# LuckyLYM/Zebra

Hardware: AMD Instinct MI355X
Metric: temporal edges/sec embedded (k=20, 2-layer) (higher is better)
Workload: dtype f64+f32

## Files before the change

zebra_amd/csrc/aggregate.hip:

```cpp
#include "common.hpp"
#include "embed_out_body.hpp"
#include "fc1_tile.hpp"

using namespace zt;
using namespace zt::dense;

namespace {

constexpr int MAX_MT = 5;
constexpr int MAX_MT_BIG = 16;
constexpr int MAX_MT_BIG_WIDE = 8;

#ifdef ZT_AGG_STAMP
__device__ unsigned long long g_agg[8];
#define AGG_STAMP(i) do { if (threadIdx.x == 0) { const long long t__ = clock64(); atomicAdd(&g_agg[i], (unsigned long long)(t__ - t_prev__)); t_prev__ = t__; } } while (0)
#else
#define AGG_STAMP(i) do { } while (0)
#endif

template <bool TAB, int MMT = MAX_MT, int NW = NTW>
__global__ __launch_bounds__(AGG_THREADS) void k_fc1_agg(FcAggArgs a, int rq, int mt_count, int lda)
{
    extern __shared__ __attribute__((aligned(16))) char smem[];
    const float *__restrict__ memory = a.memory, *__restrict__ efeat = a.efeat, *__restrict__ overlay = a.overlay;
// ... 154 lines not shown
#pragma unroll
    for (int b = 0; b < NB; ++b)
#pragma unroll
        for (int j = 0; j < 3; ++j)
            bre[b][j] = j < nrem ? bp[(size_t)b * 64 * K1p - 4 * g4 + 16 * nchunk + 4 * j + g4] : 0.f;
    const float *ap = A + (size_t)r16 * lda + 4 * g4;
    for (int kc = 0; kc < nchunk; ++kc) {
        if (kc + 1 < nchunk) {
#pragma unroll
            for (int b = 0; b < NB; ++b) bnext[b] = *reinterpret_cast<const f32x4 *>(bp + (size_t)b * 64 * K1p + 16 * (kc + 1));
        }
        f32x4 av[5];
#pragma unroll
        for (int a = 0; a < 5; ++a) av[a] = *reinterpret_cast<const f32x4 *>(ap + (size_t)a * 16 * lda + 16 * kc);
#pragma unroll
        for (int j = 0; j < 4; ++j)
#pragma unroll
            for (int a = 0; a < 5; ++a)
#pragma unroll
                for (int b = 0; b < NB; ++b)
                    acc[a][b] = __builtin_amdgcn_mfma_f32_16x16x4f32(av[a][j], bcur[b][j], acc[a][b], 0, 0, 0);
#pragma unroll
        for (int b = 0; b < NB; ++b) bcur[b] = bnext[b];
    }
    const float *ar = A + (size_t)r16 * lda + 16 * nchunk + g4;
#pragma unroll
    for (int j = 0; j < 3; ++j) {
        if (j >= nrem) break;
        float av[5];
#pragma unroll
        for (int a = 0; a < 5; ++a) av[a] = ar[(size_t)a * 16 * lda + 4 * j];
#pragma unroll
        for (int a = 0; a < 5; ++a)
#pragma unroll
            for (int b = 0; b < NB; ++b)
                acc[a][b] = __builtin_amdgcn_mfma_f32_16x16x4f32(av[a], bre[b][j], acc[a][b], 0, 0, 0);
    }
}

template <int KK>
__global__ __launch_bounds__(AGG_THREADS, 4) void k_fc1_agg_d100(
    const float *__restrict__ P, const float *__restrict__ efeat, const float *__restrict__ time_w, long long num_nodes,
    long long num_edges, int F, long long N, int lda, const int *__restrict__ nbr, const int *__restrict__ eix,
    const float *__restrict__ dt, const float *__restrict__ w, const float *__restrict__ W1p, int K1p,
    const float *__restrict__ b1, float *__restrict__ H, float *__restrict__ S, int *status)
{
    constexpr int D = 100, T = 100, DP = 112, ROWS = 80, RQ = ROWS / KK, LDH = DP + 1;
    static_assert(ROWS % KK == 0, "a tile holds whole query rows");
    extern __shared__ __attribute__((aligned(16))) char smem[];
    float *A = reinterpret_cast<float *>(smem);
    float *wn = A + (size_t)ROWS * lda;
    float *wnn = wn + ROWS;
    int *g_nb = reinterpret_cast<int *>(wnn + ROWS);
    int *g_ei = g_nb + ROWS;
    float *g_dt = reinterpret_cast<float *>(g_ei + ROWS);
    const int tid = threadIdx.x, lane = tid & 63, wave = tid >> 6;
    const int r16 = lane & 15, g4 = lane >> 4;
    const int m = blockIdx.y;
    const long long q0 = (long long)blockIdx.x * RQ;
    const int nq = (int)((N - q0) < RQ ? (N - q0) : RQ);
    const int rows = nq * KK;
    const size_t mb = ((size_t)m * N + q0) * KK;
#ifdef ZT_AGG_STAMP
    long long t_prev__ = clock64();
#endif

    float ef1 = 0.f;
    if (tid < ROWS) {
        int nb = 0, ei = 0;
        float d = 0.f, wv = 0.f;
        if (tid < rows) {
            nb = nbr[mb + tid]; ei = eix[mb + tid]; d = dt[mb + tid]; wv = w[mb + tid];
            if (nb < 0 || nb >= num_nodes || ei < 0 || ei >= num_edges) {
                atomicExch(status, ZT_ERR_RANGE);
                nb = 0; ei = 0;
            }
            if (F == 1) ef1 = efeat[ei];
        }
        g_nb[tid] = nb; g_ei[tid] = ei; g_dt[tid] = d; wn[tid] = wv;
    }
    const int cc = tid & 127;
    const float wc = cc < T ? time_w[cc] : 0.f;
    const int col0 = wave * 16 + r16;
    const float bias0 = col0 < D ? b1[col0] : 0.f, bias1 = (wave < 3 && col0 + 64 < D) ? b1[col0 + 64] : 0.f;
    __syncthreads();
    AGG_STAMP(0);

    f32x4 acc[5][2];
#pragma unroll
    for (int a = 0; a < 5; ++a) {
        const int nb4[4] = {g_nb[a * 16 + g4 * 4 + 0], g_nb[a * 16 + g4 * 4 + 1], g_nb[a * 16 + g4 * 4 + 2], g_nb[a * 16 + g4 * 4 + 3]};
#pragma unroll
        for (int j = 0; j < 4; ++j) {
            const float *pr = P + (size_t)nb4[j] * DP + col0;
            acc[a][0][j] = pr[0];
            acc[a][1][j] = pr[wave < 3 ? 64 : 0];
        }
    }
    if (tid < ROWS) {
        const int q = tid / KK;
        float my_sum = 0.f;
#pragma unroll
        for (int j = 0; j < KK; ++j) my_sum += wn[q * KK + j];
        wnn[tid] = (my_sum == 0.f) ? 0.f : wn[tid] / my_sum;
        if (tid < rows && tid - q * KK == 0) S[(size_t)m * N + q0 + q] = (my_sum == 0.f) ? 0.f : 1.f;
    }
    AGG_STAMP(1);
    if (F == 1) {
        if (tid < ROWS) A[(size_t)tid * lda] = ef1;
    } else if (F > 0) {
        constexpr int GU = 8;
        const bool vecF = (F & 3) == 0 && ((size_t)efeat & 15) == 0;
        if (vecF) {
            const int F4 = F >> 2;
            const unsigned mF4 = fastdiv_magic((unsigned)F4);
            for (int f0 = tid; f0 < ROWS * F4; f0 += AGG_THREADS * GU) {
                f32x4 v[GU];
#pragma unroll
                for (int u = 0; u < GU; ++u) {
                    const int f = f0 + u * AGG_THREADS;
                    const int g = fastdiv(f, mF4), c = f - g * F4;
                    v[u] = (f < ROWS * F4 && g < rows) ? *reinterpret_cast<const f32x4 *>(efeat + (size_t)g_ei[g] * F + 4 * c)
                                                      : f32x4{0.f, 0.f, 0.f, 0.f};
                }
#pragma unroll
                for (int u = 0; u < GU; ++u) {
                    const int f = f0 + u * AGG_THREADS;
                    const int g = fastdiv(f, mF4), c = f - g * F4;
                    if (f < ROWS * F4) *reinterpret_cast<f32x4 *>(A + (size_t)g * lda + 4 * c) = v[u];
                }
            }
        } else {
            const unsigned mF = fastdiv_magic((unsigned)F);
            for (int f0 = tid; f0 < ROWS * F; f0 += AGG_THREADS * GU) {
                float v[GU];
#pragma unroll
                for (int u = 0; u < GU; ++u) {
                    const int f = f0 + u * AGG_THREADS;
                    const int g = fastdiv(f, mF), c = f - g * F;
                    v[u] = (f < ROWS * F && g < rows) ? efeat[(size_t)g_ei[g] * F + c] : 0.f;
                }
#pragma unroll
                for (int u = 0; u < GU; ++u) {
                    const int f = f0 + u * AGG_THREADS;
                    const int g = fastdiv(f, mF), c = f - g * F;
                    if (f < ROWS * F) A[(size_t)g * lda + c] = v[u];
                }
            }
        }
    }
    {
        const int g0 = (tid >> 7) * 40;
        const bool is_cos = cc < T;
        if (is_cos || F + cc < K1p) {
            float *dst = A + (size_t)g0 * lda + F + cc;
            float xmax = 0.f;
#pragma unroll 2
            for (int i = 0; i < 40; i += 4) {
                const f32x4 d4 = *reinterpret_cast<const f32x4 *>(g_dt + g0 + i);
#pragma unroll
                for (int u = 0; u < 4; ++u) {
                    const float x = d4[u] * wc;
                    xmax = fmaxf(xmax, fabsf(x));
                    dst[(size_t)(i + u) * lda] = time_cosf_fast(x);
                }
            }
            if (!is_cos) {
                for (int i = 0; i < 40; ++i) dst[(size_t)i * lda] = 0.f;
            } else if (!(xmax < 4.0e6f)) {
                for (int i = 0; i < 40; ++i) dst[(size_t)i * lda] = time_cosf(g_dt[g0 + i] * wc);
            }
        }
    }
    AGG_STAMP(2);
    AGG_STAMP(3);
    __syncthreads();
    AGG_STAMP(4);

    {
        const float *bp = W1p + (size_t)col0 * K1p + 4 * g4;
        const int K4 = (F + T + 3) & ~3, nchunk = K4 >> 4, nrem = (K4 & 15) >> 2;
        if (wave < 3) d100_mfma<2>(A, lda, bp, K1p, nchunk, nrem, r16, g4, acc);
        else          d100_mfma<1>(A, lda, bp, K1p, nchunk, nrem, r16, g4, acc);
    }
    AGG_STAMP(5);
    __syncthreads();

    float *Hs = A;
    {
        float *hp = Hs + (size_t)(g4 * 4) * LDH + col0;
#pragma unroll
        for (int a = 0; a < 5; ++a) {
            const f32x4 w4 = *reinterpret_cast<const f32x4 *>(wnn + a * 16 + g4 * 4);
#pragma unroll
            for (int j = 0; j < 4; ++j) {
                float v = acc[a][0][j] + bias0;
                v = v > 0.f ? v : 0.f;
                hp[(size_t)(a * 16 + j) * LDH] = v * w4[j];
            }
        }
        if (wave < 3) {
#pragma unroll
            for (int a = 0; a < 5; ++a) {
                const f32x4 w4 = *reinterpret_cast<const f32x4 *>(wnn + a * 16 + g4 * 4);
#pragma unroll
                for (int j = 0; j < 4; ++j) {
                    float v1 = acc[a][1][j] + bias1;
                    v1 = v1 > 0.f ? v1 : 0.f;
                    hp[(size_t)(a * 16 + j) * LDH + 64] = v1 * w4[j];
                }
            }
        }
    }
    __syncthreads();
    AGG_STAMP(6);
    if (cc < D) {
        for (int q = tid >> 7; q < nq; q += 2) {
            const float *hq = Hs + (size_t)(q * KK) * LDH + cc;
            float s = 0.f;
#pragma unroll
            for (int j = 0; j < KK; ++j) s += hq[(size_t)j * LDH];
            H[((size_t)m * N + q0 + q) * D + cc] = s;
        }
    }
    AGG_STAMP(7);
}

#ifdef ZT_DIAG
__device__ unsigned long long g_regclk[4 * 1024];
#endif
constexpr int REG_NS = 26;
constexpr int REG_NB = 7;
constexpr int REG_FRAG_GROUPS = (REG_NB * REG_NS + 3) / 4;

__global__ void k_pack_reg_frag(const float *__restrict__ W1t, int K2p, float *__restrict__ image)
{
    const int i = blockIdx.x * blockDim.x + threadIdx.x;
    if (i >= REG_FRAG_GROUPS * 64 * 4) return;
    const int e = i & 3, lane = (i >> 2) & 63, G = i >> 8;
    const int q = 4 * G + e, b = q / REG_NS, st = q % REG_NS;
    image[i] = q < REG_NB * REG_NS ? W1t[(16 * b + (lane & 15)) * K2p + 4 * st + (lane >> 4)] : 0.f;
}

template <int KK, int DBG = 0>
__global__ __launch_bounds__(AGG_THREADS, 1) void k_fc1_agg_reg(
    const float *__restrict__ P, const float *__restrict__ efeat, const float *__restrict__ time_w, long long num_nodes,
    long long num_edges, int F, long long N, int M, const int *__restrict__ nbr, const int *__restrict__ eix,
    const float *__restrict__ dt, const float *__restrict__ w, const float *__restrict__ Wfrag,
    const float *__restrict__ b1, float *__restrict__ H, float *__restrict__ S, int *status,
    const int *gate_word, int gate_target, int *gate_latch)
{
    constexpr int D = 100, T = 100, DP = 112, ROWS = 80, RQ = ROWS / KK;
    static_assert(KK % 4 == 0 && ROWS % KK == 0, "groups of 4 rows must not straddle query rows");
    __shared__ int s_nb[AGG_WAVES][ROWS];
    __shared__ __attribute__((aligned(16))) float s_dt[AGG_WAVES][ROWS];
    __shared__ __attribute__((aligned(16))) float s_w[AGG_WAVES][ROWS];
    __shared__ float s_sum[AGG_WAVES][4];
    __shared__ __attribute__((aligned(16))) float s_ef[AGG_WAVES][ROWS * 4];
    const int lane = threadIdx.x & 63, wave = threadIdx.x >> 6;
    const int r16 = lane & 15, g4 = lane >> 4;
    int *nb_s = s_nb[wave];
    float *dt_s = s_dt[wave], *w_s = s_w[wave], *sum_s = s_sum[wave], *ef_s = s_ef[wave];
#ifdef ZT_DIAG
    const unsigned long long wall_in = DBG ? __builtin_amdgcn_s_memrealtime() : 0ull;
#endif

    float Breg[REG_NB][REG_NS];
    {
        const f32x4 *Wf = reinterpret_cast<const f32x4 *>(Wfrag) + lane;
        static_assert(REG_FRAG_GROUPS % 2 == 0, "two batches");
        constexpr int HB = REG_FRAG_GROUPS / 2;
#pragma unroll
        for (int half = 0; half < 2; ++half) {
            f32x4 v[HB];
#pragma unroll
            for (int i = 0; i < HB; ++i) v[i] = Wf[(half * HB + i) * 64];
            __builtin_amdgcn_sched_barrier(0);
#pragma unroll
            for (int i = 0; i < HB; ++i)
#pragma unroll
                for (int e = 0; e < 4; ++e) {
                    const int q = 4 * (half * HB + i) + e;
                    if (q < REG_NB * REG_NS) asm volatile("v_accvgpr_write_b32 %0, %1" : "=a"(Breg[q / REG_NS][q % REG_NS]) : "v"(v[i][e]));
                }
            __builtin_amdgcn_sched_barrier(0);
        }
    }
    float freq[REG_NS];
#pragma unroll
    for (int st = 0; st < REG_NS; ++st) {
        const int kc = 4 * st + g4 - F;
        freq[st] = (kc >= 0 && kc < T) ? time_w[kc] : 0.f;
    }
    float bias[REG_NB];
#pragma unroll
    for (int b = 0; b < REG_NB; ++b) bias[b] = (16 * b + r16) < D ? b1[16 * b + r16] : 0.f;

#ifdef ZT_DIAG
    const unsigned long long clk0 = DBG ? __builtin_amdgcn_s_memtime() : 0ull, wall0 = DBG ? __builtin_amdgcn_s_memrealtime() : 0ull;
#endif
    const long long tpm = (N + RQ - 1) / RQ;
    const long long n_tiles = tpm * M;
    const long long stride = (long long)gridDim.x * AGG_WAVES;
    long long tile = (long long)blockIdx.x * AGG_WAVES + wave;

    int pf_nb[2] = {0, 0}, pf_ei[2] = {0, 0};
    float pf_dt[2] = {0.f, 0.f}, pf_w[2] = {0.f, 0.f};
    auto fetch = [&](long long t) {
        const long long m = t / tpm, q0 = (t - m * tpm) * RQ;
        const int rows = (int)((N - q0) < RQ ? (N - q0) : RQ) * KK;
        const size_t mb = ((size_t)m * N + q0) * KK;
#pragma unroll
        for (int h = 0; h < 2; ++h) {
            const int row = h * 64 + lane;
            const bool in = row < rows && (h == 0 || lane < ROWS - 64);
            pf_nb[h] = in ? nbr[mb + row] : 0;
            pf_ei[h] = in ? eix[mb + row] : 0;
            pf_dt[h] = in ? dt[mb + row] : 0.f;
            pf_w[h] = in ? w[mb + row] : 0.f;
        }
    };
    float pf_ef[2][4] = {{0.f, 0.f, 0.f, 0.f}, {0.f, 0.f, 0.f, 0.f}};
    auto fetch_ef = [&]() {
#pragma unroll
        for (int h = 0; h < 2; ++h) {
            const int ei = pf_ei[h];
            const bool ok = ei >= 0 && ei < num_edges && (h == 0 || lane < ROWS - 64);
#pragma unroll
            for (int c = 0; c < 4; ++c) pf_ef[h][c] = (ok && c < F) ? efeat[(size_t)ei * F + c] : 0.f;
        }
    };
    member_gate_enter(gate_word, gate_target, status, gate_latch);
    if (tile < n_tiles) { fetch(tile); fetch_ef(); }

#pragma nounroll
    for (; tile < n_tiles; tile += stride) {
        const long long m = tile / tpm, q0 = (tile - m * tpm) * RQ;
        const int nq = (int)((N - q0) < RQ ? (N - q0) : RQ);
#pragma unroll
        for (int h = 0; h < 2; ++h) {
            const int row = h * 64 + lane;
            if (h == 0 || lane < ROWS - 64) {
                int nb = pf_nb[h], ei = pf_ei[h];
                if (nb < 0 || nb >= num_nodes || ei < 0 || ei >= num_edges) { atomicExch(status, ZT_ERR_RANGE); nb = 0; ei = 0; }
                nb_s[row] = nb; dt_s[row] = pf_dt[h]; w_s[row] = pf_w[h];
                *reinterpret_cast<f32x4 *>(ef_s + 4 * row) = f32x4{pf_ef[h][0], pf_ef[h][1], pf_ef[h][2], pf_ef[h][3]};
            }
        }
        wave_sync();
        if (lane < RQ) {
            f32x4 wv[KK / 4];
#pragma unroll
            for (int j = 0; j < KK / 4; ++j) wv[j] = *reinterpret_cast<const f32x4 *>(w_s + lane * KK + 4 * j);
            float sm = 0.f;
#pragma unroll
            for (int j = 0; j < KK; ++j) sm += wv[j / 4][j % 4];
            sum_s[lane] = sm;
            if (lane < nq) S[(size_t)m * N + q0 + lane] = (sm == 0.f) ? 0.f : 1.f;
        }
        wave_sync();
#pragma unroll
        for (int h = 0; h < 2; ++h) {
            const int row = h * 64 + lane;
            if (h == 0 || lane < ROWS - 64) {
                const float qs = sum_s[row / KK];
                w_s[row] = (qs == 0.f) ? 0.f : pf_w[h] / qs;
            }
        }
        wave_sync();
        const bool has_next = tile + stride < n_tiles;
        if (has_next) fetch(tile + stride);

        float Hloc[RQ][REG_NB];
#pragma unroll
        for (int q = 0; q < RQ; ++q)
#pragma unroll
            for (int b = 0; b < REG_NB; ++b) Hloc[q][b] = 0.f;

        f32x4 acc[REG_NB];
        float accv[REG_NB][4], Pv[2][REG_NB][4], wn_cur[4], wn_prv[4];
        auto load_P = [&](int x) {
            const int4 nb4 = *reinterpret_cast<const int4 *>(nb_s + x * 16 + 4 * g4);
            const float *p0 = P + (size_t)nb4.x * DP + r16, *p1 = P + (size_t)nb4.y * DP + r16,
                        *p2 = P + (size_t)nb4.z * DP + r16, *p3 = P + (size_t)nb4.w * DP + r16;
#pragma unroll
            for (int b = 0; b < REG_NB; ++b) {
                Pv[x & 1][b][0] = p0[16 * b]; Pv[x & 1][b][1] = p1[16 * b]; Pv[x & 1][b][2] = p2[16 * b]; Pv[x & 1][b][3] = p3[16 * b];
            }
        };
        if (!(DBG & 4)) { load_P(0); load_P(1); }
#pragma unroll
        for (int a = 0; a <= 5; ++a) {
            float dta = 0.f, A_next[2] = {0.f, 0.f};
            if (a > 0) {
#pragma unroll
                for (int b = 0; b < REG_NB; ++b)
#pragma unroll
                    for (int j = 0; j < 4; ++j) accv[b][j] = acc[b][j];
#pragma unroll
                for (int j = 0; j < 4; ++j) wn_prv[j] = wn_cur[j];
            }
            if (a < 5) {
                dta = dt_s[a * 16 + r16];
                const float ef = ef_s[4 * (a * 16 + r16) + (g4 & 3)];
                const f32x4 w4 = *reinterpret_cast<const f32x4 *>(w_s + a * 16 + 4 * g4);
#pragma unroll
                for (int j = 0; j < 4; ++j) wn_cur[j] = w4[j];
#pragma unroll
                for (int b = 0; b < REG_NB; ++b) acc[b] = f32x4{bias[b], bias[b], bias[b], bias[b]};
                A_next[0] = (DBG & 1) ? dta * freq[0] : time_cosf_rev(dta * freq[0]);
                A_next[1] = (DBG & 1) ? dta * freq[1] : time_cosf_rev(dta * freq[1]);
                if (g4 < F) A_next[0] = ef;
                if (a == 2 && has_next) fetch_ef();
            }
            __builtin_amdgcn_sched_barrier(0);
            const int ap = a > 0 ? a - 1 : 0;
            const int q_lo = (16 * ap) / KK, q_hi = (16 * ap + 15) / KK;
#pragma unroll
            for (int st0 = 0; st0 < REG_NS; st0 += 2) {
                if (a == 5 && st0 >= REG_NB) break;
                const float A_cur[2] = {A_next[0], A_next[1]};
                if (a < 5) {
#pragma unroll
                    for (int u = 0; u < 2; ++u)
                        if (st0 + 2 + u < REG_NS)
                            A_next[u] = (DBG & 1) ? dta * freq[st0 + 2 + u] : time_cosf_rev(dta * freq[st0 + 2 + u]);
#pragma unroll
                    for (int u = 0; u < 2; ++u)
#pragma unroll
                        for (int b = 0; b < REG_NB; ++b)
                            acc[b] = __builtin_amdgcn_mfma_f32_16x16x4f32(A_cur[u], Breg[b][st0 + u], acc[b], 0, 0, 0);
                }
#pragma unroll
                for (int u = 0; u < 2; ++u) {
                    const int st = st0 + u;
                    if (!(a > 0 && st < REG_NB)) continue;
                    const int b = st;
                    float part = 0.f;
#pragma unroll
                    for (int j = 0; j < 4; ++j) {
                        float v = accv[b][j] + ((DBG & 2) ? 0.f : Pv[ap & 1][b][j]);
                        v = v > 0.f ? v : 0.f;
                        part += (DBG & 2) ? v : v * wn_prv[j];
                    }
                    if (DBG & 2) {
                        Hloc[q_lo][b] += part;
                    } else {
                        const int pi = __float_as_int(part);
                        const auto h = __builtin_amdgcn_permlane32_swap(pi, pi, false, false);
                        const auto lo = __builtin_amdgcn_permlane16_swap(h[0], h[0], false, false);
                        const auto hi = __builtin_amdgcn_permlane16_swap(h[1], h[1], false, false);
                        const float pg[4] = {__int_as_float(lo[0]), __int_as_float(lo[1]), __int_as_float(hi[0]), __int_as_float(hi[1])};
#pragma unroll
                        for (int g = 0; g < 4; ++g) {
                            const int q = (16 * ap + 4 * g) / KK;
                            if (q < RQ) Hloc[q][b] += pg[g];
                        }
                    }
                    asm volatile("" : "+v"(Hloc[q_lo][b]));
                    if (q_hi != q_lo && q_hi < RQ) asm volatile("" : "+v"(Hloc[q_hi][b]));
                }
                if (a >= 1 && a <= 3 && st0 == REG_NB + 1 && !(DBG & 4)) load_P(a + 1);
                __builtin_amdgcn_sched_barrier(0);
            }
        }
#pragma unroll
        for (int q = 0; q < RQ; ++q) {
            if (g4 == (q & 3) && q < nq) {
                float *hrow = H + ((size_t)m * N + q0 + q) * D;
#pragma unroll
                for (int b = 0; b < REG_NB; ++b)
                    if (16 * b + r16 < D) hrow[16 * b + r16] = Hloc[q][b];
            }
        }
        wave_sync();
    }
#ifdef ZT_DIAG
    if (DBG && lane == 0 && blockIdx.x * AGG_WAVES + wave < 1024) {
        unsigned long long *o = g_regclk + 4 * (blockIdx.x * AGG_WAVES + wave);
        o[0] = __builtin_amdgcn_s_memtime() - clk0; o[1] = wall0; o[2] = __builtin_amdgcn_s_memrealtime();
        o[3] = wall_in;
    }
#endif
}


constexpr int EO3_NT = 7, EO3_KC = 7, EO3_DP = 112, EO3_LDY = 116;
constexpr int EO3_FRAG = EO3_NT * EO3_KC * 256;

__device__ __forceinline__ void eo3_fill(float *Wl, const float *__restrict__ Wp, int tid)
{
    constexpr int PER = (EO3_NT * EO3_KC * 64 + 255) / 256;
    f32x4 v[PER];
#pragma unroll
    for (int q = 0; q < PER; ++q) {
        const int idx = tid + q * 256, frag = idx >> 6, ln = idx & 63;
        const int b = frag / EO3_KC, c = frag - b * EO3_KC;
        v[q] = idx < EO3_NT * EO3_KC * 64
                   ? *reinterpret_cast<const f32x4 *>(Wp + (size_t)(16 * b + (ln & 15)) * EO3_DP + 16 * c + 4 * (ln >> 4))
                   : f32x4{0.f, 0.f, 0.f, 0.f};
    }
#pragma unroll
    for (int q = 0; q < PER; ++q) {
        const int idx = tid + q * 256;
        if (idx < EO3_NT * EO3_KC * 64) reinterpret_cast<f32x4 *>(Wl)[idx] = v[q];
    }
}

template <int HG>
__global__ __launch_bounds__(AGG_THREADS, 1) void k_embed_out3(
    const float *__restrict__ memory, long long num_nodes, const int *__restrict__ nodes, long long N, int D, int M,
    const float *__restrict__ H, const float *__restrict__ S, const float *__restrict__ fc2_p,
    const float *__restrict__ fc2_b, const float *__restrict__ fc1s_p, const float *__restrict__ fc1s_b,
    const float *__restrict__ fc2s_p, const float *__restrict__ fc2s_b, float *__restrict__ out, int *status, int n_src)
{
    extern __shared__ __attribute__((aligned(16))) char smem[];
    float *W0 = reinterpret_cast<float *>(smem);
    const int tid = threadIdx.x, lane = tid & 63, wave = tid >> 6, r16 = lane & 15, g4 = lane >> 4;
    const int OW = D * (M + 1);
    const long long tiles = (N + 15) / 16;
    const f32x4 zero4 = {0.f, 0.f, 0.f, 0.f};
    bool cin[EO3_KC];
#pragma unroll
    for (int c = 0; c < EO3_KC; ++c) cin[c] = 16 * c + 4 * g4 < D;
    const f32x4 *Wf0 = reinterpret_cast<const f32x4 *>(W0) + lane;

    if ((int)blockIdx.x < n_src) {
        float *W1 = W0 + EO3_FRAG;
        float *Y = W1 + EO3_FRAG + wave * 16 * EO3_LDY;
        eo3_fill(W0, fc1s_p, tid);
        eo3_fill(W1, fc2s_p, tid);
        float b1v[EO3_NT], b2v[EO3_NT];
#pragma unroll
        for (int b = 0; b < EO3_NT; ++b) {
            b1v[b] = 16 * b + r16 < D ? fc1s_b[16 * b + r16] : 0.f;
            b2v[b] = 16 * b + r16 < D ? fc2s_b[16 * b + r16] : 0.f;
        }
        const f32x4 *Wf1 = reinterpret_cast<const f32x4 *>(W1) + lane;
        const long long stride = (long long)n_src * AGG_WAVES;
        long long t = (long long)blockIdx.x * AGG_WAVES + wave;
        auto node_of = [&](long long tt) -> int { return (tt < tiles && tt * 16 + r16 < N) ? nodes[tt * 16 + r16] : -1; };
        auto rows_of = [&](int nd, f32x4 (&a)[EO3_KC]) {
            const bool ok = nd >= 0 && nd < num_nodes;
#pragma unroll
            for (int c = 0; c < EO3_KC; ++c)
                a[c] = (ok && cin[c]) ? *reinterpret_cast<const f32x4 *>(memory + (size_t)nd * D + 16 * c + 4 * g4) : zero4;
        };
        int nd_cur = node_of(t), nd_nxt = node_of(t + stride);
        f32x4 a[EO3_KC], an[EO3_KC];
        if (t < tiles) rows_of(nd_cur, a);
        __syncthreads();
        for (; t < tiles; t += stride) {
            const long long r0 = t * 16;
            if (r0 + r16 < N && (nd_cur < 0 || nd_cur >= num_nodes)) atomicExch(status, ZT_ERR_RANGE);
            rows_of(nd_nxt, an);
            nd_cur = nd_nxt;
            nd_nxt = node_of(t + 2 * stride);
            f32x4 acc1[EO3_NT];
#pragma unroll
            for (int b = 0; b < EO3_NT; ++b) acc1[b] = zero4;
#pragma unroll
            for (int c = 0; c < EO3_KC; ++c) {
                f32x4 w[EO3_NT];
#pragma unroll
                for (int b = 0; b < EO3_NT; ++b) w[b] = Wf0[(b * EO3_KC + c) * 64];
#pragma unroll
                for (int j = 0; j < 4; ++j)
#pragma unroll
                    for (int b = 0; b < EO3_NT; ++b) acc1[b] = __builtin_amdgcn_mfma_f32_16x16x4f32(a[c][j], w[b][j], acc1[b], 0, 0, 0);
            }
#pragma unroll
            for (int b = 0; b < EO3_NT; ++b)
#pragma unroll
                for (int j = 0; j < 4; ++j) {
                    const float v = acc1[b][j] + b1v[b];
                    Y[(4 * g4 + j) * EO3_LDY + 16 * b + r16] = (16 * b + r16 < D && v > 0.f) ? v : 0.f;
                }
            wave_sync();
            f32x4 acc[EO3_NT];
#pragma unroll
            for (int b = 0; b < EO3_NT; ++b) acc[b] = zero4;
#pragma unroll
            for (int c = 0; c < EO3_KC; ++c) {
                const f32x4 y = *reinterpret_cast<const f32x4 *>(Y + r16 * EO3_LDY + 16 * c + 4 * g4);
                f32x4 w[EO3_NT];
#pragma unroll
                for (int b = 0; b < EO3_NT; ++b) w[b] = Wf1[(b * EO3_KC + c) * 64];
#pragma unroll
                for (int j = 0; j < 4; ++j)
#pragma unroll
                    for (int b = 0; b < EO3_NT; ++b) acc[b] = __builtin_amdgcn_mfma_f32_16x16x4f32(y[j], w[b][j], acc[b], 0, 0, 0);
            }
#pragma unroll
            for (int b = 0; b < EO3_NT; ++b) {
                const int col = 16 * b + r16;
                if (col < D) {
#pragma unroll
                    for (int j = 0; j < 4; ++j)
                        if (r0 + 4 * g4 + j < N) out[(size_t)(r0 + 4 * g4 + j) * OW + col] = acc[b][j] + b2v[b];
                }
            }
            wave_sync();
#pragma unroll
            for (int c = 0; c < EO3_KC; ++c) a[c] = an[c];
        }
        return;
    }
    eo3_fill(W0, fc2_p, tid);
    float b2v[EO3_NT];
#pragma unroll
    for (int b = 0; b < EO3_NT; ++b) b2v[b] = 16 * b + r16 < D ? fc2_b[16 * b + r16] : 0.f;
    const long long units = tiles * M;
    const long long stride = (long long)((int)gridDim.x - n_src) * AGG_WAVES;
    long long u = (long long)((int)blockIdx.x - n_src) * AGG_WAVES + wave;
    constexpr int GQ = HG == 1 ? 1 : 5;
    auto rows_of = [&](long long uu, int q0, f32x4 (&g)[GQ][EO3_KC]) {
        const long long m = uu / tiles, r = (uu - m * tiles) * 16 + r16;
        const bool rin = uu < units && r < N;
        const float *hp = H + (((size_t)m * N + (rin ? r : 0)) * HG + q0) * D + 4 * g4;
#pragma unroll
        for (int q = 0; q < GQ; ++q)
#pragma unroll
            for (int c = 0; c < EO3_KC; ++c) g[q][c] = (rin && cin[c]) ? *reinterpret_cast<const f32x4 *>(hp + (size_t)q * D + 16 * c) : zero4;
    };
    f32x4 gn[GQ][EO3_KC];
    if (HG == 1) rows_of(u, 0, gn);
    __syncthreads();
    for (; u < units; u += stride) {
        const long long m = u / tiles, r0 = (u - m * tiles) * 16;
        f32x4 a[EO3_KC];
        if (HG == 1) {
#pragma unroll
            for (int c = 0; c < EO3_KC; ++c) a[c] = gn[0][c];
        } else {
#pragma nounroll
            for (int q0 = 0; q0 < HG; q0 += GQ) {
                rows_of(u, q0, gn);
#pragma unroll
                for (int c = 0; c < EO3_KC; ++c) {
                    if (q0 == 0) a[c] = gn[0][c]; else a[c] += gn[0][c];
#pragma unroll
                    for (int q = 1; q < GQ; ++q) a[c] += gn[q][c];
                }
            }
        }
        float sv[4];
#pragma unroll
        for (int j = 0; j < 4; ++j) sv[j] = r0 + 4 * g4 + j < N ? S[(size_t)m * N + r0 + 4 * g4 + j] : 0.f;
        if (HG == 1) rows_of(u + stride, 0, gn);
        f32x4 acc[EO3_NT];
#pragma unroll
        for (int b = 0; b < EO3_NT; ++b) acc[b] = zero4;
#pragma unroll
        for (int c = 0; c < EO3_KC; ++c) {
            f32x4 w[EO3_NT];
#pragma unroll
            for (int b = 0; b < EO3_NT; ++b) w[b] = Wf0[(b * EO3_KC + c) * 64];
#pragma unroll
            for (int j = 0; j < 4; ++j)
#pragma unroll
                for (int b = 0; b < EO3_NT; ++b) acc[b] = __builtin_amdgcn_mfma_f32_16x16x4f32(a[c][j], w[b][j], acc[b], 0, 0, 0);
        }
#pragma unroll
        for (int b = 0; b < EO3_NT; ++b) {
            const int col = 16 * b + r16;
            if (col < D) {
#pragma unroll
                for (int j = 0; j < 4; ++j)
                    if (r0 + 4 * g4 + j < N) out[(size_t)(r0 + 4 * g4 + j) * OW + (size_t)D * (m + 1) + col] = acc[b][j] + b2v[b] * sv[j];
            }
        }
    }
}

template <int NW = NTW>
__global__ __launch_bounds__(AGG_THREADS) void k_project_rows(const float *__restrict__ memory, long long num_nodes,
                                                              int D, const float *__restrict__ Wm_p,
                                                              const int *__restrict__ rows, const int *__restrict__ count,
                                                              long long n_max, float *__restrict__ P)
{
    extern __shared__ __attribute__((aligned(16))) char smem[];
    const int Dp = (D + 15) / 16 * 16, ldx = Dp + 4, NT = Dp / 16;
    float *X = reinterpret_cast<float *>(smem);
    int *rid = reinterpret_cast<int *>(X + OUT_ROWS * ldx);
    const int tid = threadIdx.x, lane = tid & 63, wave = tid >> 6;
    const int r16 = lane & 15, g4 = lane >> 4;
    const long long r0 = (long long)blockIdx.x * OUT_ROWS;
    long long n = n_max;
    if (count != nullptr) { const long long c = *count; n = c < n ? c : n; }
    if (r0 >= n) return;
    if (tid < OUT_ROWS) {
        long long v = -1;
        if (r0 + tid < n) v = rows != nullptr ? (long long)rows[r0 + tid] : r0 + tid;
        rid[tid] = (v >= 0 && v < num_nodes) ? (int)v : -1;
    }
    __syncthreads();
    const unsigned mL = fastdiv_magic((unsigned)ldx);
    for (int f = tid; f < OUT_ROWS * ldx; f += AGG_THREADS) {
        const int g = fastdiv(f, mL), c = f - g * ldx;
        X[f] = (rid[g] >= 0 && c < D) ? memory[(size_t)rid[g] * D + c] : 0.f;
    }
    __syncthreads();
    f32x4 acc[OUT_MT][NW];
    small_gemm(X, ldx, Wm_p, Dp, NT, wave, lane, acc);
#pragma unroll
    for (int b = 0; b < NW; ++b) {
        const int col = (wave + b * AGG_WAVES) * 16 + r16;
        if (col >= Dp) continue;
#pragma unroll
        for (int a = 0; a < OUT_MT; ++a)
#pragma unroll
            for (int j = 0; j < 4; ++j) {
                const int g = a * 16 + g4 * 4 + j;
                if (rid[g] >= 0) P[(size_t)rid[g] * Dp + col] = acc[a][b][j];
            }
    }
}

struct EmbedPlan {
    int Dp, K1p, lda, mt, rq;
    size_t lds;
    int K2p, lda2, mt2, rq2;
    size_t lds2;
    size_t off_w1p, off_H, off_S, off_fc2t, off_fc1st, off_fc2st, off_w1t, off_wm, off_wl, off_wfrag, total;
    int hg;
};

bool tile_shape(int Kp, int Dp, int k, int T, int *lda_out, int *mt_out, int *rq_out, size_t *lds_out, int max_mt = MAX_MT)
{
    const int lda = Kp + 4;
    int mt = max_mt;
    while (mt > 1 && ((size_t)mt * 16 * lda * 4 + (size_t)mt * 16 * 16) > (size_t)AGG_LDS_BUDGET) --mt;
    int rq = (mt * 16) / k;
    if (rq < 1) {
        mt = (k + 15) / 16;
        rq = 1;
        if (mt > max_mt || ((size_t)mt * 16 * lda * 4 + (size_t)mt * 16 * 16) > (size_t)AGG_LDS_BUDGET) return false;
    }
    mt = (rq * k + 15) / 16;
    if ((size_t)mt * 16 * (Dp + 1) * 4 > (size_t)mt * 16 * lda * 4) return false;
    *lda_out = lda; *mt_out = mt; *rq_out = rq;
    *lds_out = (size_t)mt * 16 * lda * 4 + (size_t)mt * 16 * 16 + (size_t)T * 4;
    return true;
}

bool split_fits(int D, int F, int T, int k) { return k <= ZT_MAX_K_WIDE && fc1_agg_split_rows(D, F, T) > 0; }

bool make_plan(int64_t N, int D, int F, int T, int M, int k, EmbedPlan &p)
{
    if (!width_supported(D)) return false;
    const int K1 = D + F + T;
    p.Dp = round_up(D, 16);
    p.K1p = round_up(K1, 16);
    const bool big = k > MAX_MT * 16;
    const int max_mt = big ? (p.Dp > 16 * NTW * AGG_WAVES ? MAX_MT_BIG_WIDE : MAX_MT_BIG) : MAX_MT;
    const bool full_ok = tile_shape(p.K1p, p.Dp, k, T, &p.lda, &p.mt, &p.rq, &p.lds, max_mt);
    if (!full_ok) { p.mt = 0; p.rq = 1; p.lda = p.K1p + 4; p.lds = 0; }
    p.K2p = round_up(F + T, 16);
    p.mt2 = 0;
    if (!(full_ok || big) || !tile_shape(p.K2p, p.Dp, k, T, &p.lda2, &p.mt2, &p.rq2, &p.lds2, max_mt)) p.mt2 = 0;
    if (p.mt == 0 && p.mt2 == 0 && !split_fits(D, F, T, k)) return false;
    size_t o = 0;
    auto take = [&](size_t bytes) { size_t r = o; o += (bytes + 255) & ~(size_t)255; return r; };
    p.off_w1p = take((size_t)p.Dp * p.K1p * 4);
    p.off_fc2t = take((size_t)p.Dp * p.Dp * 4);
    p.off_fc1st = take((size_t)p.Dp * p.Dp * 4);
    p.off_fc2st = take((size_t)p.Dp * p.Dp * 4);
    p.off_w1t = take((size_t)p.Dp * p.K2p * 4);
    p.off_wm = take((size_t)p.Dp * p.Dp * 4);
    p.hg = fc1_agg_wide_supported(D, F, T, k) ? k / 4 : 1;
    p.off_wl = take(p.hg > 1 ? fc1_agg_wide_weight_bytes() : 0);
    p.off_wfrag = take((size_t)REG_FRAG_GROUPS * 64 * 4 * 4);
    p.off_H = take((size_t)M * N * D * 4 * p.hg);
    p.off_S = take((size_t)M * N * 4);
    p.total = o;
    return true;
}

// ... 399 lines not shown
```

Before: 14.07 million.

## Software-pipeline register aggregation kernel: stagger acc handoff, split P loads, drop divisions

Restructures the register-resident fc1 aggregation loop into a compile-time-unrolled per-subtile lambda. The next subtile's time encoding and row reads are computed during the current MFMA chain, accumulators are handed off piecewise, and neighbor P loads are spread across stages. Per-tile 64-bit divisions for m/q0 are replaced by incremental tile/row-base counters, and edge-feature loads become branchless, using unsigned range checks with clamped indices. The aim is to hide latency and cut scalar/ALU overhead, at the cost of more complex scheduling and possible register pressure.

```diff
diff --git a/zebra_amd/csrc/aggregate.hip b/zebra_amd/csrc/aggregate.hip
--- a/zebra_amd/csrc/aggregate.hip
+++ b/zebra_amd/csrc/aggregate.hip
@@ -480,14 +480,23 @@
     const long long tpm = (N + RQ - 1) / RQ;
     const long long n_tiles = tpm * M;
     const long long stride = (long long)gridDim.x * AGG_WAVES;
-    long long tile = (long long)blockIdx.x * AGG_WAVES + wave;
+    long long tile = (long long)blockIdx.x * AGG_WAVES + __builtin_amdgcn_readfirstlane(wave);
+    long long cur_t = tile, cur_rb = tile * RQ;
+    const long long rb_wrap = N - tpm * RQ;
+    if (tile < n_tiles)
+        while (cur_t >= tpm) { cur_t -= tpm; cur_rb += rb_wrap; }
+    long long nxt_t = cur_t, nxt_rb = cur_rb;
+    auto advance = [&](long long &t, long long &rb) {
+        t += stride; rb += stride * RQ;
+        while (t >= tpm) { t -= tpm; rb += rb_wrap; }
+    };
 
     int pf_nb[2] = {0, 0}, pf_ei[2] = {0, 0};
     float pf_dt[2] = {0.f, 0.f}, pf_w[2] = {0.f, 0.f};
-    auto fetch = [&](long long t) {
-        const long long m = t / tpm, q0 = (t - m * tpm) * RQ;
+    auto fetch = [&](long long t, long long rb) {
+        const long long q0 = t * RQ;
         const int rows = (int)((N - q0) < RQ ? (N - q0) : RQ) * KK;
-        const size_t mb = ((size_t)m * N + q0) * KK;
+        const size_t mb = (size_t)rb * KK;
 #pragma unroll
         for (int h = 0; h < 2; ++h) {
             const int row = h * 64 + lane;
@@ -499,30 +508,36 @@
         }
     };
     float pf_ef[2][4] = {{0.f, 0.f, 0.f, 0.f}, {0.f, 0.f, 0.f, 0.f}};
-    auto fetch_ef = [&]() {
-#pragma unroll
-        for (int h = 0; h < 2; ++h) {
-            const int ei = pf_ei[h];
-            const bool ok = ei >= 0 && ei < num_edges && (h == 0 || lane < ROWS - 64);
-#pragma unroll
-            for (int c = 0; c < 4; ++c) pf_ef[h][c] = (ok && c < F) ? efeat[(size_t)ei * F + c] : 0.f;
-        }
+    const float *ef_src = (F > 0 && num_edges > 0) ? efeat : time_w;
+    const int ef_ld = (F > 0 && num_edges > 0) ? F : 0;
+    const unsigned nn_u = num_nodes > 0x7fffffffLL ? 0x80000000u : (num_nodes > 0 ? (unsigned)num_nodes : 0u);
+    const unsigned ne_u = num_edges > 0x7fffffffLL ? 0x80000000u : (num_edges > 0 ? (unsigned)num_edges : 0u);
+    auto fetch_ef = [&](int h) {
+        const unsigned ei = (unsigned)pf_ei[h] < ne_u ? (unsigned)pf_ei[h] : 0u;
+        const float *row = ef_src + (size_t)ei * ef_ld;
+#pragma unroll
+        for (int c = 0; c < 4; ++c) pf_ef[h][c] = row[c < ef_ld ? c : (ef_ld > 0 ? ef_ld - 1 : 0)];
     };
     member_gate_enter(gate_word, gate_target, status, gate_latch);
-    if (tile < n_tiles) { fetch(tile); fetch_ef(); }
+    if (tile < n_tiles) { fetch(cur_t, cur_rb); fetch_ef(0); fetch_ef(1); }
 
 #pragma nounroll
     for (; tile < n_tiles; tile += stride) {
-        const long long m = tile / tpm, q0 = (tile - m * tpm) * RQ;
+        const long long q0 = cur_t * RQ;
         const int nq = (int)((N - q0) < RQ ? (N - q0) : RQ);
+        float *const s_row = S + (size_t)cur_rb;
+        float *const h_row = H + (size_t)cur_rb * D;
 #pragma unroll
         for (int h = 0; h < 2; ++h) {
             const int row = h * 64 + lane;
             if (h == 0 || lane < ROWS - 64) {
-                int nb = pf_nb[h], ei = pf_ei[h];
-                if (nb < 0 || nb >= num_nodes || ei < 0 || ei >= num_edges) { atomicExch(status, ZT_ERR_RANGE); nb = 0; ei = 0; }
+                int nb = pf_nb[h];
+                const int ei = pf_ei[h];
+                const bool e_in = (unsigned)ei < ne_u;
+                if ((unsigned)nb >= nn_u || !e_in) { atomicExch(status, ZT_ERR_RANGE); nb = 0; }
                 nb_s[row] = nb; dt_s[row] = pf_dt[h]; w_s[row] = pf_w[h];
-                *reinterpret_cast<f32x4 *>(ef_s + 4 * row) = f32x4{pf_ef[h][0], pf_ef[h][1], pf_ef[h][2], pf_ef[h][3]};
+                *reinterpret_cast<f32x4 *>(ef_s + 4 * row) = f32x4{(e_in && 0 < F) ? pf_ef[h][0] : 0.f, (e_in && 1 < F) ? pf_ef[h][1] : 0.f,
+                                                                   (e_in && 2 < F) ? pf_ef[h][2] : 0.f, (e_in && 3 < F) ? pf_ef[h][3] : 0.f};
             }
         }
         wave_sync();
@@ -534,7 +549,7 @@
 #pragma unroll
             for (int j = 0; j < KK; ++j) sm += wv[j / 4][j % 4];
             sum_s[lane] = sm;
-            if (lane < nq) S[(size_t)m * N + q0 + lane] = (sm == 0.f) ? 0.f : 1.f;
+            if (lane < nq) s_row[lane] = (sm == 0.f) ? 0.f : 1.f;
         }
         wave_sync();
 #pragma unroll
@@ -547,7 +562,7 @@
         }
         wave_sync();
         const bool has_next = tile + stride < n_tiles;
-        if (has_next) fetch(tile + stride);
+        if (has_next) { advance(nxt_t, nxt_rb); fetch(nxt_t, nxt_rb); }
 
         float Hloc[RQ][REG_NB];
 #pragma unroll
@@ -556,41 +571,47 @@
             for (int b = 0; b < REG_NB; ++b) Hloc[q][b] = 0.f;
 
         f32x4 acc[REG_NB];
-        float accv[REG_NB][4], Pv[2][REG_NB][4], wn_cur[4], wn_prv[4];
-        auto load_P = [&](int x) {
+        float accv[REG_NB][4], Pv[2][REG_NB][4], wn[2][4];
+        float dta = 0.f, dtn = 0.f, efn = 0.f, A_next[2] = {0.f, 0.f};
+        auto take_acc = [&](int b) {
+            __builtin_amdgcn_sched_barrier(0);
+#pragma unroll
+            for (int j = 0; j < 4; ++j) { accv[b][j] = acc[b][j]; asm volatile("" : "+v"(accv[b][j])); }
+            __builtin_amdgcn_sched_barrier(0);
+        };
+        auto read_rows = [&](int x) {
+            dtn = dt_s[x * 16 + r16];
+            efn = ef_s[4 * (x * 16 + r16) + (g4 & 3)];
+            const f32x4 w4 = *reinterpret_cast<const f32x4 *>(w_s + x * 16 + 4 * g4);
+#pragma unroll
+            for (int j = 0; j < 4; ++j) wn[x & 1][j] = w4[j];
+        };
+        auto time_enc = [&](float d, int st) { return (DBG & 1) ? d * freq[st] : time_cosf_rev(d * freq[st]); };
+        const float *p0 = P, *p1 = P, *p2 = P, *p3 = P;
+        auto load_P_rows = [&](int x) {
             const int4 nb4 = *reinterpret_cast<const int4 *>(nb_s + x * 16 + 4 * g4);
-            const float *p0 = P + (size_t)nb4.x * DP + r16, *p1 = P + (size_t)nb4.y * DP + r16,
-                        *p2 = P + (size_t)nb4.z * DP + r16, *p3 = P + (size_t)nb4.w * DP + r16;
-#pragma unroll
-            for (int b = 0; b < REG_NB; ++b) {
-                Pv[x & 1][b][0] = p0[16 * b]; Pv[x & 1][b][1] = p1[16 * b]; Pv[x & 1][b][2] = p2[16 * b]; Pv[x & 1][b][3] = p3[16 * b];
-            }
+            p0 = P + (size_t)nb4.x * DP + r16; p1 = P + (size_t)nb4.y * DP + r16;
+            p2 = P + (size_t)nb4.z * DP + r16; p3 = P + (size_t)nb4.w * DP + r16;
         };
-        if (!(DBG & 4)) { load_P(0); load_P(1); }
-#pragma unroll
-        for (int a = 0; a <= 5; ++a) {
-            float dta = 0.f, A_next[2] = {0.f, 0.f};
-            if (a > 0) {
-#pragma unroll
-                for (int b = 0; b < REG_NB; ++b)
-#pragma unroll
-                    for (int j = 0; j < 4; ++j) accv[b][j] = acc[b][j];
-#pragma unroll
-                for (int j = 0; j < 4; ++j) wn_prv[j] = wn_cur[j];
-            }
-            if (a < 5) {
-                dta = dt_s[a * 16 + r16];
-                const float ef = ef_s[4 * (a * 16 + r16) + (g4 & 3)];
-                const f32x4 w4 = *reinterpret_cast<const f32x4 *>(w_s + a * 16 + 4 * g4);
-#pragma unroll
-                for (int j = 0; j < 4; ++j) wn_cur[j] = w4[j];
-#pragma unroll
-                for (int b = 0; b < REG_NB; ++b) acc[b] = f32x4{bias[b], bias[b], bias[b], bias[b]};
-                A_next[0] = (DBG & 1) ? dta * freq[0] : time_cosf_rev(dta * freq[0]);
-                A_next[1] = (DBG & 1) ? dta * freq[1] : time_cosf_rev(dta * freq[1]);
-                if (g4 < F) A_next[0] = ef;
-                if (a == 2 && has_next) fetch_ef();
-            }
+        auto load_P_part = [&](int x, int b) {
+            Pv[x & 1][b][0] = p0[16 * b]; Pv[x & 1][b][1] = p1[16 * b]; Pv[x & 1][b][2] = p2[16 * b]; Pv[x & 1][b][3] = p3[16 * b];
+        };
+        constexpr int LP0 = REG_NB + 1;
+        if (!(DBG & 4)) {
+            load_P_rows(0);
+#pragma unroll
+            for (int b = 0; b < REG_NB; ++b) load_P_part(0, b);
+        }
+        auto m_tile = [&](auto A_) __attribute__((always_inline)) {
+            constexpr int a = decltype(A_)::value;
+            if (a == 0) {
+                read_rows(0);
+                A_next[0] = time_enc(dtn, 0);
+                A_next[1] = time_enc(dtn, 1);
+                if (g4 < F) A_next[0] = efn;
+            }
+            if (a == 5) { take_acc(REG_NB - 2); take_acc(REG_NB - 1); }
+            dta = dtn;
             __builtin_amdgcn_sched_barrier(0);
             const int ap = a > 0 ? a - 1 : 0;
             const int q_lo = (16 * ap) / KK, q_hi = (16 * ap + 15) / KK;
@@ -599,15 +620,23 @@
                 if (a == 5 && st0 >= REG_NB) break;
                 const float A_cur[2] = {A_next[0], A_next[1]};
                 if (a < 5) {
+                    if (a < 4 && st0 == 18) read_rows(a + 1);
+#pragma unroll
+                    for (int u = 0; u < 2; ++u) {
+                        if (st0 + 2 + u < REG_NS) A_next[u] = time_enc(dta, st0 + 2 + u);
+                        else if (a < 4) A_next[u] = time_enc(dtn, st0 + 2 + u - REG_NS);
+                    }
+                    if (st0 + 2 >= REG_NS && a < 4 && g4 < F) A_next[0] = efn;
 #pragma unroll
                     for (int u = 0; u < 2; ++u)
-                        if (st0 + 2 + u < REG_NS)
-                            A_next[u] = (DBG & 1) ? dta * freq[st0 + 2 + u] : time_cosf_rev(dta * freq[st0 + 2 + u]);
-#pragma unroll
-                    for (int u = 0; u < 2; ++u)
-#pragma unroll
-                        for (int b = 0; b < REG_NB; ++b)
-                            acc[b] = __builtin_amdgcn_mfma_f32_16x16x4f32(A_cur[u], Breg[b][st0 + u], acc[b], 0, 0, 0);
+#pragma unroll
+                        for (int b = 0; b < REG_NB; ++b) {
+                            const int st = st0 + u;
+                            const f32x4 c = st == 0 ? f32x4{bias[b], bias[b], bias[b], bias[b]} : acc[b];
+                            if (a > 0 && st == 0 && b >= 1 && b <= 2) take_acc(REG_NB - 3 + b);
+                            acc[b] = __builtin_amdgcn_mfma_f32_16x16x4f32(A_cur[u], Breg[b][st], c, 0, 0, 0);
+                            if (st == REG_NS - 1 && b >= 2) take_acc(b - 2);
+                        }
                 }
 #pragma unroll
                 for (int u = 0; u < 2; ++u) {
@@ -619,7 +648,7 @@
                     for (int j = 0; j < 4; ++j) {
                         float v = accv[b][j] + ((DBG & 2) ? 0.f : Pv[ap & 1][b][j]);
                         v = v > 0.f ? v : 0.f;
-                        part += (DBG & 2) ? v : v * wn_prv[j];
+                        part += (DBG & 2) ? v : v * wn[ap & 1][j];
                     }
                     if (DBG & 2) {
                         Hloc[q_lo][b] += part;
@@ -638,20 +667,30 @@
                     asm volatile("" : "+v"(Hloc[q_lo][b]));
                     if (q_hi != q_lo && q_hi < RQ) asm volatile("" : "+v"(Hloc[q_hi][b]));
                 }
-                if (a >= 1 && a <= 3 && st0 == REG_NB + 1 && !(DBG & 4)) load_P(a + 1);
+                const int lp = st0 - (a == 0 ? 0 : LP0);
+                if (a <= 3 && lp >= 0 && lp < REG_NB && !(DBG & 4)) {
+                    if (lp == 0) load_P_rows(a + 1);
+                    load_P_part(a + 1, lp);
+                    if (lp + 1 < REG_NB) load_P_part(a + 1, lp + 1);
+                }
+                if (a == 2 && (st0 == 16 || st0 == 18)) fetch_ef((st0 - 16) / 2);
                 __builtin_amdgcn_sched_barrier(0);
             }
-        }
+        };
+        m_tile(std::integral_constant<int, 0>{}); m_tile(std::integral_constant<int, 1>{}); m_tile(std::integral_constant<int, 2>{});
+        m_tile(std::integral_constant<int, 3>{}); m_tile(std::integral_constant<int, 4>{});
+        m_tile(std::integral_constant<int, 5>{});
 #pragma unroll
         for (int q = 0; q < RQ; ++q) {
             if (g4 == (q & 3) && q < nq) {
-                float *hrow = H + ((size_t)m * N + q0 + q) * D;
+                float *hrow = h_row + q * D;
 #pragma unroll
                 for (int b = 0; b < REG_NB; ++b)
                     if (16 * b + r16 < D) hrow[16 * b + r16] = Hloc[q][b];
             }
         }
         wave_sync();
+        cur_t = nxt_t; cur_rb = nxt_rb;
     }
 #ifdef ZT_DIAG
     if (DBG && lane == 0 && blockIdx.x * AGG_WAVES + wave < 1024) {
```

Result: faster. 14.33 million, median of 5 (+1.8%).
